# aagbotemi/zk-cryptography

Hardware: AMD Instinct MI355X
Metric: field-evals/s (sumcheck 2^24) + MSM points/s (KZG 2^20) per BASELINE.json; value = the sumcheck prover's field-evals/s, the MSM half is under "msm" (higher is better)
Workload: dtype u32; 1 GPU; 24-var multilinear sumcheck prover (poly_sum + prove), BLS12-381 Fr; field=BLS12-381 Fr (255-bit Montgomery, 8 x u32 limbs); G1 over Fq (381-bit), evals_per_gpu=16777216, exchanges_per_prove=0

## Files before the change

### zk-cryptography_amd/csrc/multifold_kernels.hpp

```cpp
#pragma once
#include "sumcheck_kernels.hpp"
#include "wide_acc.hpp"

namespace zk {

constexpr int MF_MAX_LOGK = 8;
constexpr int MF_CAP_LOGK = 9;

static __global__ __launch_bounds__(MLE_BLOCK) void chunk_sums_kernel(const uint64_t* __restrict__ in, uint32_t chunk,
                                                                      uint64_t* __restrict__ partials) {
    __shared__ Fr red[MLE_BLOCK / 64];
    const uint64_t* base = in + 4 * (size_t)blockIdx.x * chunk;
    Fr s = Fr::zero();
    for (uint32_t j = threadIdx.x; j < chunk; j += 4 * MLE_BLOCK) {
        Fr v[4];
#pragma unroll
        for (int u = 0; u < 4; ++u) v[u] = (j + u * MLE_BLOCK < chunk) ? load_fr(base, j + u * MLE_BLOCK) : Fr::zero();
#pragma unroll
        for (int u = 0; u < 4; ++u) s = s + v[u];
    }
    s = block_reduce_fr(s, red);
    if (threadIdx.x == 0) store_fr(partials, blockIdx.x, s);
}

// ... 37 lines not shown
                                                                         uint64_t* __restrict__ out_mont, uint64_t* __restrict__ out_canon) {
    __shared__ Fr red[MLE_BLOCK / 64];
    const uint64_t* base = in + 4 * (size_t)blockIdx.x * group;
    Fr s = Fr::zero();
    for (uint32_t j = threadIdx.x; j < group; j += 4 * MLE_BLOCK) {
        Fr v[4];
#pragma unroll
        for (int u = 0; u < 4; ++u) v[u] = (j + u * MLE_BLOCK < group) ? load_fr(base, j + u * MLE_BLOCK) : Fr::zero();
#pragma unroll
        for (int u = 0; u < 4; ++u) s = s + v[u];
    }
    s = block_reduce_fr(s, red);
    if (threadIdx.x == 0) {
        if (out_mont) store_fr(out_mont, blockIdx.x, s);
        if (out_canon) store_fr(out_canon, blockIdx.x, fr_from_mont_outlined(s));
    }
}

constexpr int TREE_MAX_LOG = 10;

struct SmallArgs {
    const uint64_t* src;
    uint32_t group;
    uint32_t stride;
    uint32_t canon;
    uint32_t log_n;
    uint32_t n_rounds;
    uint32_t round0;
    uint32_t first;
    FrArg claimed;
    const uint64_t* d_claimed;
    uint64_t* weights_out;
    uint64_t* final_out;
    long long host_delta;
};

constexpr int SMALL_BLOCK = 512;

static __global__ __launch_bounds__(SMALL_BLOCK) void sumcheck_small_kernel(SmallArgs a, SumcheckDev* st,
                                                                            uint64_t* __restrict__ round_polys,
                                                                            uint64_t* __restrict__ challenges) {
    extern __shared__ __attribute__((aligned(16))) unsigned char zk_dyn_lds[];
    __builtin_amdgcn_s_setprio(3);
    ZK_STAMP_AT(0, 40 + a.round0, 0);
    const uint32_t n = 1u << a.log_n;
    Fr* tree0 = reinterpret_cast<Fr*>(zk_dyn_lds);
    Fr* tree1 = tree0 + 2 * n;
    const uint32_t w_all = a.weights_out ? (1u << a.n_rounds) : 0u;
    Fr* w0 = tree1 + n;
    Fr* w1 = w0 + ((a.n_rounds & 1) ? w_all / 2 : w_all);
    const bool grouped = a.group != 0 && a.stride == 0;
    Fr* scratch = w0 + w_all + w_all / 2 + 1;
    Fr* e_sh = scratch + (grouped ? SMALL_BLOCK : 0);
    Fr* r_sh = e_sh + 4;
    if (a.host_delta && a.round0) {
        for (uint32_t i = threadIdx.x; i < 12 * a.round0 + 4; i += SMALL_BLOCK) {
            const uint64_t* p = i < 4 ? st->sum + i : i < 4 + 8 * a.round0 ? round_polys + (i - 4) : challenges + (i - 4 - 8 * a.round0);
            *const_cast<uint64_t*>(p + a.host_delta) = *p;
        }
    }
    if (a.group == 0) {
        for (uint32_t j = threadIdx.x; j < n; j += SMALL_BLOCK) {
            const Fr v = load_fr(a.src, j);
            tree0[n + j] = a.canon ? v : fr_from_mont_outlined(v);
        }
    } else if (a.stride != 0) {
        for (uint32_t j = threadIdx.x; j < n; j += SMALL_BLOCK) {
            Fr s = load_fr(a.src, j);
            for (uint32_t g = 1; g < a.group; g += 8) {
                Fr v[8];
#pragma unroll
                for (int u = 0; u < 8; ++u) if (g + u < a.group) v[u] = load_fr(a.src, (size_t)(g + u) * a.stride + j);
#pragma unroll
                for (int u = 0; u < 8; ++u) if (g + u < a.group) s = s + v[u];
            }
            tree0[n + j] = a.canon ? s : fr_from_mont_outlined(s);
        }
    } else {
        const uint32_t total = n * a.group;
        const uint32_t run = total > (uint32_t)SMALL_BLOCK ? total / SMALL_BLOCK : 1;
        if (threadIdx.x * run < total) {
            Fr s = Fr::zero();
            for (uint32_t g = 0; g < run; ++g) s = s + load_fr(a.src, (size_t)threadIdx.x * run + g);
            scratch[threadIdx.x] = s;
        }
        __syncthreads();
        const uint32_t tpe = a.group / run;
        for (uint32_t j = threadIdx.x; j < n; j += SMALL_BLOCK) {
            Fr s = scratch[j * tpe];
            for (uint32_t g = 1; g < tpe; ++g) s = s + scratch[j * tpe + g];
            tree0[n + j] = a.canon ? s : fr_from_mont_outlined(s);
        }
    }
    if (threadIdx.x == 0 && a.weights_out) {
        Fr one32;
        constexpr uint32_t c[8] = {0xcaaf6b13u, 0x355094eau, 0x69a568efu, 0xf6b10cb3u, 0x40cc3869u, 0xe2c926a6u, 0xed269aadu, 0x736a6d3bu};
#pragma unroll
        for (int i = 0; i < 8; ++i) one32.l[i] = c[i];
        w0[0] = one32;
    }
    __syncthreads();
    for (uint32_t lvl = a.log_n; lvl > 1;) {
        const uint32_t step = lvl - 1 < 3 ? lvl - 1 : 3;
        const uint32_t groups = 1u << (lvl - step);
        for (uint32_t g = threadIdx.x; g < groups; g += SMALL_BLOCK) {
            Fr v[8];
            const uint32_t cnt0 = 1u << step;
#pragma unroll
            for (int i = 0; i < 8; ++i) if ((uint32_t)i < cnt0) v[i] = tree0[(1u << lvl) + g * cnt0 + i];
#pragma unroll
            for (int sft = 1; sft <= 3; ++sft) {
                if ((uint32_t)sft <= step) {
                    const uint32_t cnt = cnt0 >> sft;
#pragma unroll
                    for (int i = 0; i < 4; ++i) {
                        if ((uint32_t)i < cnt) {
                            v[i] = v[2 * i] + v[2 * i + 1];
                            tree0[(1u << (lvl - sft)) + g * cnt + i] = v[i];
                        }
                    }
                }
            }
        }
        __syncthreads();
        lvl -= step;
    }
    const uint32_t wave = threadIdx.x >> 6;
    const bool wave0 = wave == 0;
    uint32_t* kw1 = reinterpret_cast<uint32_t*>(r_sh + 2);
    uint32_t* kw2 = kw1 + 64;
    uint32_t* dig_sh = kw2 + 64;
    uint32_t* flags = dig_sh + 16;
    if (threadIdx.x >= 64 && threadIdx.x < 66 && a.log_n >= 2)
        e_sh[threadIdx.x - 64] = (tree0[6 + threadIdx.x - 64] - tree0[4 + threadIdx.x - 64]).to_mont();
    if (threadIdx.x == 0) {
        flags[0] = 0; flags[1] = 0;
        uint32_t pre[8];
        if (a.first) {
            const Fr sum_c = (a.first == 2) ? fr_from_mont_outlined(fr_from_arg(a.claimed))
                           : (a.first == 3) ? fr_from_mont_outlined(load_fr(a.d_claimed, 0)) : tree0[2] + tree0[3];
#pragma unroll
            for (int i = 0; i < 8; ++i) pre[i] = sum_c.l[7 - i];
        } else {
#pragma unroll
            for (int i = 0; i < 8; ++i) pre[i] = st->transcript.buf[i];
        }
#pragma unroll
        for (int i = 0; i < 8; ++i) dig_sh[8 + i] = pre[i];
    }
    __syncthreads();
    Fr lo = tree0[2], hi = tree0[3];
    uint32_t depth = a.log_n, round = a.round0, n_w = 1;
    ZK_STAMP_AT(0, 40 + a.round0, 1);
    const uint32_t word = threadIdx.x & 15;
    auto schedule_block1 = [&](const uint32_t* prefix, const Fr& lo_c, uint32_t it) {
        const uint32_t w = word < 8 ? prefix[word] : fr_limb_by_lane(lo_c, 15 - word);
        sha256_schedule_rows_to_lds(w, kw1, flags, 4 * it, 1, threadIdx.x < 64 + 16);
    };
    auto schedule_block2 = [&](const Fr& hi_c, uint32_t it) {
        const uint32_t w = word < 8 ? fr_limb_by_lane(hi_c, 7 - word) : (word == 8 ? 0x80000000u : word == 15 ? 96u * 8u : 0u);
        sha256_schedule_rows_to_lds(w, kw2, flags + 1, 4 * it, 0, threadIdx.x < 128 + 16);
    };
    if (a.n_rounds) {
        if (wave == 1) schedule_block1(dig_sh + 8, lo, 0);
        if (wave == 2) schedule_block2(hi, 0);
    }
    uint32_t digest[8];
    constexpr uint32_t FIRST_HELPER = 192, N_HELPERS = SMALL_BLOCK - FIRST_HELPER - 64, OUT_WAVE = 4;
    if (wave == OUT_WAVE) __builtin_amdgcn_s_setprio(0);
    for (uint32_t it = 0; it < a.n_rounds; ++it) {
        Fr* told = (it & 1) ? tree1 : tree0;
        Fr* tnew = (it & 1) ? tree0 : tree1;
        Fr* wold = (it & 1) ? w1 : w0;
        Fr* wnew = (it & 1) ? w0 : w1;
        Fr* eold = e_sh + 2 * (it & 1);
        Fr* enew = e_sh + 2 * ((it & 1) ^ 1);
        const bool absorb_sum = a.first && it == 0;
        if (wave0) {
            ZK_STAMP_AT(0, round, 0);
            uint32_t h[8] = {0x6a09e667u, 0xbb67ae85u, 0x3c6ef372u, 0xa54ff53au, 0x510e527fu, 0x9b05688cu, 0x1f83d9abu, 0x5be0cd19u};
            uint32_t blk[16];
            const uint32_t* pre = dig_sh + 8 * ((it + 1) & 1);
#pragma unroll
            for (int i = 0; i < 8; ++i) { blk[i] = pre[i]; blk[8 + i] = lo.l[7 - i]; }
            ShaSplit sp;
            sp.init();
            uint32_t hs[4];
            sp.split(h, hs);
            sha256_compress_kw_split(sp, hs, blk, kw1, flags, 4 * it);
            ZK_STAMP_AT(0, round, 1);
            sha256_compress_kw_split(sp, hs, nullptr, kw2, flags + 1, 4 * it);
            sp.join(hs, h);
            ZK_STAMP_AT(0, round, 2);
#pragma unroll
            for (int i = 0; i < 8; ++i) digest[i] = h[i];
            Fr c;
#pragma unroll
            for (int i = 0; i < 8; ++i) c.l[i] = h[7 - i];
            c.reduce_once();
            c.reduce_once();
            if (threadIdx.x == 0) {
                r_sh[it & 1] = c;
#pragma unroll
                for (int i = 0; i < 8; ++i) dig_sh[8 * (it & 1) + i] = h[i];
            }
        }
        ZK_STAMP_AT(0, round, 3);
        ZK_STAMP_AT(SMALL_BLOCK - 1, round, 6);
        ZK_STAMP_AT(64, round, 7);
        __syncthreads();
        ZK_STAMP_AT(0, round, 4);
        const Fr c = r_sh[it & 1];
        if (wave0) {
            if (depth >= 2) {
                const uint32_t q = threadIdx.x & 1;
                Fr v = told[4 + q] + fr_mul_outlined(c, eold[q]);
                lo = shfl_fr(v, 0);
                hi = shfl_fr(v, 1);
            }
            ZK_STAMP_AT(0, round, 5);
        } else if (wave <= 2) {
            if (it + 1 < a.n_rounds && depth >= 2) {
                const uint32_t q = wave - 1;
                const Fr v = told[4 + q] + fr_mul_outlined(c, eold[q]);
                if (wave == 1) schedule_block1(dig_sh + 8 * (it & 1), v, it + 1);
                else schedule_block2(v, it + 1);
            }
        } else {
            const Fr r = fr_to_mont_outlined(c);
            const uint32_t helper = wave == OUT_WAVE ? N_HELPERS : wave < OUT_WAVE ? threadIdx.x - FIRST_HELPER : threadIdx.x - FIRST_HELPER - 64;
            if (threadIdx.x == 64 * OUT_WAVE) {
                Fr lo_m = told[2].to_mont(), hi_m = told[3].to_mont();
                if (absorb_sum) {
                    Fr sum_m = (a.first == 2) ? fr_from_arg(a.claimed) : (a.first == 3) ? load_fr(a.d_claimed, 0) : lo_m + hi_m;
                    store_fr(st->sum, 0, sum_m);
                    if (a.host_delta) store_fr(st->sum + a.host_delta, 0, sum_m);
                }
                store_fr(round_polys, 2 * (size_t)round, lo_m);
                store_fr(round_polys, 2 * (size_t)round + 1, hi_m);
                store_fr(challenges, round, r);
                if (a.host_delta) {
                    store_fr(round_polys + a.host_delta, 2 * (size_t)round, lo_m);
                    store_fr(round_polys + a.host_delta, 2 * (size_t)round + 1, hi_m);
                    store_fr(challenges + a.host_delta, round, r);
                }
            }
            const uint32_t nodes = 1u << (depth - 1);
            if (helper >= N_HELPERS - 2 && helper < N_HELPERS && depth >= 3) {
                const uint32_t q = 4 + (helper - (N_HELPERS - 2));
                Fr va = told[q + 4] + r * (told[q + 8] - told[q + 4]);
                Fr vb = told[q + 6] + r * (told[q + 10] - told[q + 6]);
                tnew[q] = va;
                tnew[q + 2] = vb;
                enew[helper - (N_HELPERS - 2)] = (vb - va).to_mont();
            }
            for (uint32_t q = 1 + helper; q < 2 * nodes && helper < N_HELPERS; q += N_HELPERS) {
                if (depth >= 3 && q >= 4 && q < 8) continue;
                const uint32_t p = 1u << (31 - __builtin_clz(q));
                tnew[q] = told[q + p] + r * (told[q + 2 * p] - told[q + p]);
            }
            if (a.weights_out) {
                for (uint32_t b = helper; b < n_w && helper < N_HELPERS; b += N_HELPERS) {
                    Fr w1v = wold[b] * r;
                    wnew[2 * b + 1] = w1v;
                    wnew[2 * b] = wold[b] - w1v;
                }
            }
        }
        n_w <<= 1;
        --depth;
        ++round;
    }
    ZK_STAMP_AT(0, 40 + a.round0, 2);
    __syncthreads();
    if (threadIdx.x == 0 && a.n_rounds) {
        Transcript tr;
        tr.init();
        tr.commit_words8(digest);
        tr.store(&st->transcript);
    }

    if (a.weights_out) {
        Fr* w = (a.n_rounds & 1) ? w1 : w0;
        for (uint32_t b = threadIdx.x; b < n_w; b += SMALL_BLOCK) store_fr(a.weights_out, b, w[b]);
    }
    if (a.final_out) {
        Fr* t = (a.n_rounds & 1) ? tree1 : tree0;
        const uint32_t cnt = 1u << depth;
        for (uint32_t j = threadIdx.x; j < cnt; j += SMALL_BLOCK) store_fr(a.final_out, j, t[cnt + j].to_mont());
    }
}
__host__ __device__ constexpr size_t small_lds_bytes(uint32_t log_n, int weight_rounds, bool grouped) {
    return ((size_t)3 * ((size_t)1 << log_n) + (weight_rounds >= 0 ? 3 * ((size_t)1 << weight_rounds) / 2 : 0u) + 1 +
            (grouped ? SMALL_BLOCK : 0) + 4 + 2) * 32 + (64 + 64 + 16 + 2) * 4;
}

static __global__ __launch_bounds__(MLE_BLOCK) void eq_weights_kernel(PtsArg pts, uint32_t first, uint32_t k,
                                                                      uint64_t* __restrict__ out) {
    const uint32_t b = blockIdx.x * MLE_BLOCK + threadIdx.x;
    if (b >= (1u << k)) return;
    Fr w;
    constexpr uint32_t c[8] = {0xcaaf6b13u, 0x355094eau, 0x69a568efu, 0xf6b10cb3u, 0x40cc3869u, 0xe2c926a6u, 0xed269aadu, 0x736a6d3bu};
#pragma unroll
    for (int i = 0; i < 8; ++i) w.l[i] = c[i];
    const Fr one = Fr::one();
    for (uint32_t i = 0; i < k; ++i) {
        Fr r = fr_from_pts(pts, first + i);
        if (!((b >> (k - 1 - i)) & 1)) r = one - r;
        w = w * r;
    }
    store_fr(out, b, w);
}

static __global__ __launch_bounds__(MLE_BLOCK) void eval_weights_kernel(PtsArg pts, uint32_t k1, uint32_t k2, uint32_t s, uint64_t* __restrict__ w1,
                                                                        uint64_t* __restrict__ wa, uint64_t* __restrict__ wb) {
    size_t b = (size_t)blockIdx.x * MLE_BLOCK + threadIdx.x;
    const size_t n1 = (size_t)1 << k1, na = (size_t)1 << (k2 - s), nb = (size_t)1 << s;
    uint32_t k, first;
    uint64_t* out;
    Fr w = Fr::one();
    if (b < n1) {
        k = k1; first = 0; out = w1;
        constexpr uint32_t c[8] = {0xcaaf6b13u, 0x355094eau, 0x69a568efu, 0xf6b10cb3u, 0x40cc3869u, 0xe2c926a6u, 0xed269aadu, 0x736a6d3bu};
#pragma unroll
        for (int i = 0; i < 8; ++i) w.l[i] = c[i];
    } else if (b < n1 + na) {
        b -= n1; k = k2 - s; first = k1; out = wa;
    } else if (b < n1 + na + nb) {
        b -= n1 + na; k = s; first = k1 + k2 - s; out = wb;
    } else {
        return;
    }
    const Fr one = Fr::one();
    for (uint32_t i = 0; i < k; ++i) {
        Fr r = fr_from_pts(pts, first + i);
        if (!((b >> (k - 1 - i)) & 1)) r = one - r;
        w = w * r;
    }
    store_fr(out, b, w);
}
static __global__ __launch_bounds__(MLE_BLOCK) void sum_records_kernel(const uint64_t* __restrict__ records, uint32_t n, uint64_t* __restrict__ out) {
    __shared__ Fr red[MLE_BLOCK / 64];
    Fr s = Fr::zero();
    for (uint32_t i = threadIdx.x; i < n; i += 4 * MLE_BLOCK) {
        Fr v[4];
#pragma unroll
        for (int u = 0; u < 4; ++u) v[u] = (i + u * MLE_BLOCK < n) ? load_fr(records, i + u * MLE_BLOCK) : Fr::zero();
// ... 11 lines not shown
                                                                uint64_t* __restrict__ partials) {
    constexpr int TG = 64 / G;
    extern __shared__ __attribute__((aligned(16))) unsigned char zk_dyn_lds[];
    Fr* w_lds = reinterpret_cast<Fr*>(zk_dyn_lds);
    Fr* part = w_lds + (1u << k);
    const uint32_t n_terms = 1u << k;
    for (uint32_t b = threadIdx.x; b < n_terms; b += blockDim.x) w_lds[b] = load_fr(weights, b);
    __syncthreads();
    const uint32_t lane = threadIdx.x & 63;
    const uint32_t wave = threadIdx.x >> 6;
    const uint32_t n_waves = blockDim.x >> 6;
    const uint32_t slice = wave * TG + lane / G;
    const uint32_t per = n_terms / (n_waves * TG);
    const uint32_t oj = lane % G;
    const size_t j = (size_t)blockIdx.x * G + oj;
    WideAcc acc;
    acc.clear();
    const uint32_t b0 = slice * per;
    const uint64_t* p = in + 4 * ((size_t)b0 * m + j);
    const size_t row = 4 * m;
    for (uint32_t t = 0; t < per; t += DEPTH) {
        Fr v[DEPTH];
#pragma unroll
        for (int u = 0; u < DEPTH; ++u) if (t + u < per) v[u] = NT ? load_fr_nt(p + (size_t)(t + u) * row) : load_fr(p + (size_t)(t + u) * row, 0);
#pragma unroll
        for (int u = 0; u < DEPTH; ++u) if (t + u < per) acc.mac(w_lds[b0 + t + u], v[u]);
    }
    Fr o = wide_reduce(acc.lo, acc.hi);
#pragma unroll
    for (int d = 32; d >= G; d >>= 1) o = o + shfl_down_fr(o, d);
    if (wave != 0 && lane < G) part[(wave - 1) * G + lane] = o;
    __syncthreads();
    if (wave == 0) {
        if (lane < G) {
            for (uint32_t w2 = 1; w2 < n_waves; ++w2) o = o + part[(w2 - 1) * G + lane];
            store_fr(out, j, o);
        } else {
            o = Fr::zero();
        }
        Fr s = wave_reduce_fr(o);
        if (lane == 0) store_fr(partials, blockIdx.x, s);
    }
}

static __global__ __launch_bounds__(MLE_BLOCK) void slice_sums_kernel(const uint64_t* __restrict__ in, uint32_t ny, uint32_t m,
                                                               uint64_t* __restrict__ out) {
    const uint32_t j = blockIdx.x * MLE_BLOCK + threadIdx.x;
    if (j >= m) return;
    Fr s = load_fr(in, j);
    for (uint32_t y = 1; y < ny; ++y) s = s + load_fr(in, (size_t)y * m + j);
    store_fr(out, j, fr_to_mont_outlined(s));
}

constexpr int BF_BLOCK = 1024;
static __global__ __launch_bounds__(BF_BLOCK) void blockfold_kernel(const uint64_t* __restrict__ in, uint32_t m, uint32_t log_ow,
                                                                    uint32_t per, const uint64_t* __restrict__ weights,
                                                                    uint64_t* __restrict__ partial) {
    __shared__ Fr part[BF_BLOCK];
    const uint32_t ow = 1u << log_ow, sl_cnt = BF_BLOCK >> log_ow;
    const uint32_t o = threadIdx.x & (ow - 1), sl = threadIdx.x >> log_ow;
    const uint32_t c = blockIdx.x * ow + o;
    const uint32_t b0 = (blockIdx.y * sl_cnt + sl) * per;
    WideAcc acc;
    acc.clear();
    for (uint32_t u = 0; u < per; u += 2) {
        Fr v0 = load_fr(in, (size_t)(b0 + u) * m + c), w0 = load_fr(weights, b0 + u);
        Fr v1 = v0, w1 = w0;
        const bool two = u + 1 < per;
        if (two) { v1 = load_fr(in, (size_t)(b0 + u + 1) * m + c); w1 = load_fr(weights, b0 + u + 1); }
        acc.mac(w0, v0);
        if (two) acc.mac(w1, v1);
    }
    part[threadIdx.x] = wide_reduce(acc.lo, acc.hi);
    __syncthreads();
    for (uint32_t half = sl_cnt >> 1; half >= 1; half >>= 1) {
        if (sl < half) part[threadIdx.x] = part[threadIdx.x] + part[threadIdx.x + (half << log_ow)];
        __syncthreads();
    }
    if (sl == 0) store_fr(partial, (size_t)blockIdx.y * m + c, fr_from_mont_outlined(part[o]));
}

}
```

### zk-cryptography_amd/csrc/transcript.hpp

```cpp
#pragma once
#include "fp.hpp"

namespace zk {

struct Sha256State {
    uint32_t h[8];
    uint32_t buf[16];
    uint32_t fill;
    uint32_t pad_;
    uint64_t len;
};

__device__ __forceinline__ uint32_t rotr32(uint32_t x, int n) { return __builtin_rotateright32(x, n); }

static __constant__ uint32_t SHA256_K[64] = {
    0x428a2f98, 0x71374491, 0xb5c0fbcf, 0xe9b5dba5, 0x3956c25b, 0x59f111f1, 0x923f82a4, 0xab1c5ed5,
    0xd807aa98, 0x12835b01, 0x243185be, 0x550c7dc3, 0x72be5d74, 0x80deb1fe, 0x9bdc06a7, 0xc19bf174,
    0xe49b69c1, 0xefbe4786, 0x0fc19dc6, 0x240ca1cc, 0x2de92c6f, 0x4a7484aa, 0x5cb0a9dc, 0x76f988da,
    0x983e5152, 0xa831c66d, 0xb00327c8, 0xbf597fc7, 0xc6e00bf3, 0xd5a79147, 0x06ca6351, 0x14292967,
    0x27b70a85, 0x2e1b2138, 0x4d2c6dfc, 0x53380d13, 0x650a7354, 0x766a0abb, 0x81c2c92e, 0x92722c85,
    0xa2bfe8a1, 0xa81a664b, 0xc24b8b70, 0xc76c51a3, 0xd192e819, 0xd6990624, 0xf40e3585, 0x106aa070,
    0x19a4c116, 0x1e376c08, 0x2748774c, 0x34b0bcb5, 0x391c0cb3, 0x4ed8aa4a, 0x5b9cca4f, 0x682e6ff3,
    0x748f82ee, 0x78a5636f, 0x84c87814, 0x8cc70208, 0x90befffa, 0xa4506ceb, 0xbef9a3f7, 0xc67178f2};

// ... 315 lines not shown
    }
    sp.join(hs, h);
}

__device__ __forceinline__ void sha256_compress_wave(uint32_t (&h)[8], const uint32_t (&blk)[16], uint32_t* lds) {
    const uint32_t i = threadIdx.x & 15;
    uint32_t w = blk[0];
#pragma unroll
    for (int k = 1; k < 16; ++k) w = i == (uint32_t)k ? blk[k] : w;
    sha256_schedule_rows_to_lds(w, lds, nullptr, 0u, 0u, (threadIdx.x & 63) < 16);
    __builtin_amdgcn_fence(__ATOMIC_ACQ_REL, "workgroup");
    ShaSplit sp;
    sp.init();
    uint32_t hs[4];
    sp.split(h, hs);
    sha256_rounds_block_split(sp, hs, lds);
    sp.join(hs, h);
    __builtin_amdgcn_fence(__ATOMIC_ACQ_REL, "workgroup");
}

__device__ __noinline__ Fr fr_mul_outlined(Fr a, Fr b) { return a * b; }
__device__ __noinline__ Fr fr_from_mont_outlined(Fr a) {
    uint32_t x[9];
#pragma unroll
    for (int i = 0; i < 8; ++i) x[i] = a.l[i];
    x[8] = 0;
#pragma unroll
    for (int i = 0; i < 8; ++i) {
        const uint32_t m = FrParams::mul_inv(x[0]);
        uint64_t c = ((uint64_t)m * FrParams::p(0) + x[0]) >> 32;
#pragma unroll
        for (int j = 1; j < 8; ++j) {
            uint64_t s = (uint64_t)m * FrParams::p(j) + x[j] + c;
            x[j - 1] = (uint32_t)s;
            c = s >> 32;
        }
        uint64_t s = (uint64_t)x[8] + c;
        x[7] = (uint32_t)s;
        x[8] = (uint32_t)(s >> 32);
    }
    Fr r;
#pragma unroll
    for (int i = 0; i < 8; ++i) r.l[i] = x[i];
    r.reduce_once();
    return r;
}
__device__ __forceinline__ Fr fr_to_mont_outlined(const Fr& a) {
    Fr r2;
#pragma unroll
    for (int i = 0; i < Fr::N; ++i) r2.l[i] = FrParams::r2(i);
    return fr_mul_outlined(a, r2);
}

struct Transcript {
    uint32_t h[8];
    uint32_t buf[16];
    uint32_t fill_words;
    uint64_t len;

    __device__ __forceinline__ void init() {
        h[0] = 0x6a09e667; h[1] = 0xbb67ae85; h[2] = 0x3c6ef372; h[3] = 0xa54ff53a;
        h[4] = 0x510e527f; h[5] = 0x9b05688c; h[6] = 0x1f83d9ab; h[7] = 0x5be0cd19;
        fill_words = 0;
        len = 0;
#pragma unroll
        for (int i = 0; i < 16; ++i) buf[i] = 0;
    }
    __device__ __forceinline__ void load(const Sha256State* s) {
#pragma unroll
        for (int i = 0; i < 8; ++i) h[i] = s->h[i];
#pragma unroll
        for (int i = 0; i < 16; ++i) buf[i] = s->buf[i];
        fill_words = s->fill >> 2;
        len = s->len;
    }
    __device__ __forceinline__ void store(Sha256State* s) const {
#pragma unroll
        for (int i = 0; i < 8; ++i) s->h[i] = h[i];
#pragma unroll
        for (int i = 0; i < 16; ++i) s->buf[i] = buf[i];
        s->fill = fill_words << 2;
        s->len = len;
    }
    __device__ __forceinline__ void commit_words8(const uint32_t (&wds)[8]) {
        if (fill_words == 0) {
#pragma unroll
            for (int i = 0; i < 8; ++i) buf[i] = wds[i];
            fill_words = 8;
        } else {
#pragma unroll
            for (int i = 0; i < 8; ++i) buf[8 + i] = wds[i];
            sha256_compress(h, buf);
            fill_words = 0;
        }
        len += 32;
    }
    __device__ __forceinline__ void commit_canonical(const Fr& c) {
        uint32_t wds[8];
#pragma unroll
        for (int i = 0; i < 8; ++i) wds[i] = c.l[7 - i];
        commit_words8(wds);
    }
    __device__ __forceinline__ void commit_fr(const Fr& v_mont) {
        Fr c = fr_from_mont_outlined(v_mont);
        uint32_t wds[8];
#pragma unroll
// ... 63 lines not shown
```

### zk-cryptography_amd/csrc/zkhip.hip

```cpp
#include "../../include/zkhip.h"

#include <hip/hip_runtime.h>

#include <algorithm>
#include <cstdio>
#include <cstdlib>
#include <cstring>
#include <map>
#include <string>
#include <vector>

#include "ctx.hpp"
#include "host_util.hpp"
#include "mle_kernels.hpp"
#include "sumcheck_kernels.hpp"
#include "multifold_kernels.hpp"
#include "mfma_fold.hpp"
#include "tunables.hpp"

using namespace zk;

static int g_last_hip = 0;
extern "C" int zkhip_version(void) { return 1; }

// ... 431 lines not shown
extern "C" int zkhip_circuit_add_mult_mle(zkhip_ctx* c, const uint8_t* h_gate_type, const uint32_t* h_in0, const uint32_t* h_in1,
                                          size_t n_gates, uint32_t layer_index, uint64_t* d_add, uint64_t* d_mul) {
    if (!c || !d_add || !d_mul || (n_gates && (!h_gate_type || !h_in0 || !h_in1))) return ZKHIP_ERR_ARG;
    if (layer_index > 12) return ZKHIP_ERR_SHAPE;
    const size_t size = zkhip_gkr_mle_size(layer_index);
    const uint32_t shift = layer_index + 1;
    for (size_t g = 0; g < n_gates; ++g) {
        const size_t idx = (g << (2 * shift)) | ((size_t)h_in0[g] << shift) | h_in1[g];
        if (idx >= size) return ZKHIP_ERR_INDEX;
    }
    ZK_TRY(c->activate());
    ZK_HIP(c, hipMemsetAsync(d_add, 0, 32 * size, c->stream));
    ZK_HIP(c, hipMemsetAsync(d_mul, 0, 32 * size, c->stream));
    if (n_gates == 0) return ZKHIP_OK;
    uint32_t* d_gates = nullptr;
    ZK_TRY(upload_gates(c, h_gate_type, h_in0, h_in1, n_gates, &d_gates));
    hipLaunchKernelGGL(wiring_ones_kernel, dim3(mle_grid(n_gates)), dim3(MLE_BLOCK), 0, c->stream, d_gates, n_gates, shift, d_add, d_mul);
    ZK_HIP(c, hipGetLastError());
    ZK_HIP(c, hipStreamSynchronize(c->stream));
    return ZKHIP_OK;
}

static inline uint32_t stage_k(size_t cur_n) {
    if (cur_n <= ((size_t)1 << TREE_MAX_LOG)) return 0;
    const uint32_t lg = log2_exact(cur_n);
    uint32_t k = lg - 8;
    if (k > MF_MAX_LOGK) k = MF_MAX_LOGK;
    return k;
}
static inline uint32_t overlapped_min_log() {
    static const uint32_t v = (uint32_t)zk::env::read(zk::env::OVERLAP_MIN_LOG); return v;
}
static inline bool overlapped_plan(size_t n) { return is_pow2(n) && n >= ((size_t)1 << overlapped_min_log()) && n <= ((size_t)1 << 24); }
static inline bool overlapped_shard(size_t n) { return is_pow2(n) && n >= ((size_t)1 << 19) && n <= ((size_t)1 << 24); }
static inline uint32_t overlapped_k2(size_t n) { return std::min<uint32_t>(TREE_MAX_LOG, log2_exact(n) - 8 - 3); }
extern "C" int zkhip_sumcheck_plan_log_blocks(size_t n) {
    if (!is_pow2(n)) return 0;
    return overlapped_plan(n) ? (int)(log2_exact(n) - 8) : (int)stage_k(n);
}

static int launch_small(zkhip_ctx* c, const SmallArgs& a, SumcheckDev* st, uint64_t* d_rp, uint64_t* d_ch, size_t min_lds = 0,
                        hipStream_t stream = nullptr) {
    if (!stream) stream = c->stream;
    if (a.log_n > (uint32_t)TREE_MAX_LOG || a.n_rounds > a.log_n) return ZKHIP_ERR_SHAPE;
    const size_t lds = std::max(small_lds_bytes(a.log_n, a.weights_out ? (int)a.n_rounds : -1, a.group != 0 && a.stride == 0), min_lds);
    if (lds > 160 * 1024) return ZKHIP_ERR_SHAPE;
    ZK_TRY(c->allow_big_lds((const void*)sumcheck_small_kernel, 160 * 1024));
    ProfScope ps(c, "sumcheck_small", 0.0, stream);
    hipLaunchKernelGGL(sumcheck_small_kernel, dim3(1), dim3(SMALL_BLOCK), lds, stream, a, st, d_rp, d_ch);
    ZK_HIP(c, hipGetLastError());
    return ZKHIP_OK;
}

struct BlockfoldShape { uint32_t log_ow, per, ny; };
static inline bool blockfold_shape(uint32_t m, uint32_t k, BlockfoldShape* sh) {
    const uint32_t log_m = log2_exact(m);
    sh->log_ow = std::max<uint32_t>(std::min<uint32_t>(log_m, 5), k < 10 ? 10 - k : 0);
    if (sh->log_ow > log_m) return false;
    const uint32_t sl_cnt = (uint32_t)BF_BLOCK >> sh->log_ow;
    const uint32_t terms = 1u << k;
    sh->per = std::min<uint32_t>(4, terms / sl_cnt);
    sh->ny = terms / (sh->per * sl_cnt);
    return true;
}
static int launch_blockfold(zkhip_ctx* c, hipStream_t stream, const uint64_t* in, uint32_t m, uint32_t k, const uint64_t* d_w,
                            uint64_t* d_partial, uint32_t* n_slices) {
    BlockfoldShape sh;
    if (!blockfold_shape(m, k, &sh)) return ZKHIP_ERR_SHAPE;
    const uint32_t log_ow = sh.log_ow, per = sh.per, ny = sh.ny, terms = 1u << k;
    ProfScope ps(c, "blockfold", 32.0 * (double)m * terms, stream);
    hipLaunchKernelGGL(blockfold_kernel, dim3(m >> log_ow, ny), dim3(BF_BLOCK), 0, stream, in, m, log_ow, per, d_w, d_partial);
    ZK_HIP(c, hipGetLastError());
    *n_slices = ny;
    return ZKHIP_OK;
}
static int launch_fine_sums(zkhip_ctx* c, const uint64_t* d_evals, size_t n, uint32_t lb, uint64_t* d_fine, uint64_t* d_chunk,
                            hipStream_t stream = nullptr) {
    if (!stream) stream = c->stream;
    const size_t blk = n >> lb, n_chunks = n / FINE_CHUNK;
    uint64_t* first = blk == (size_t)FINE_CHUNK ? d_fine : d_chunk;
    {
        ProfScope ps(c, "fine_sums", 32.0 * (double)n, stream);
        static const size_t lds = (size_t)zk::env::read(zk::env::FINE_LDS);
        if (lds > 64 * 1024) ZK_TRY(c->allow_big_lds((const void*)fine_sums_kernel, 158 * 1024));
        hipLaunchKernelGGL(fine_sums_kernel, dim3((unsigned)((n_chunks + 7) / 8)), dim3(MLE_BLOCK), lds, stream, d_evals, n_chunks, first);
    }
    if (first != d_fine)
        hipLaunchKernelGGL(group_sums_wg_kernel, dim3(1u << lb), dim3(MLE_BLOCK), 0, stream, first, (uint32_t)(blk / FINE_CHUNK), d_fine, (uint64_t*)nullptr);
    ZK_HIP(c, hipGetLastError());
    return ZKHIP_OK;
}

static int block_sums_impl(zkhip_ctx* c, const uint64_t* d_evals, size_t n, uint32_t log_blocks, uint64_t* d_out, uint64_t* h_total, bool want_total);
extern "C" int zkhip_mle_block_sums(zkhip_ctx* c, const uint64_t* d_evals, size_t n, uint32_t log_blocks,
                                    uint64_t* d_out, uint64_t* h_total) {
    return block_sums_impl(c, d_evals, n, log_blocks, d_out, h_total, true);
}
extern "C" int zkhip_mle_block_sums_deferred(zkhip_ctx* c, const uint64_t* d_evals, size_t n, uint32_t log_blocks, uint64_t* d_out) {
    return block_sums_impl(c, d_evals, n, log_blocks, d_out, nullptr, false);
}
extern "C" int zkhip_mle_block_sums_total(zkhip_ctx* c, uint64_t* d_block_sums, uint32_t log_blocks, uint64_t* h_total) {
    if (!c || !d_block_sums || !h_total || log_blocks > 16) return ZKHIP_ERR_ARG;
    ZK_TRY(c->activate());
    const uint32_t hi = log_blocks / 2, lo = log_blocks - hi;
    uint64_t* tmp = c->small_u64(ZK_SMALL_PARTIALS);
    hipLaunchKernelGGL(group_sums_wg_kernel, dim3(1u << hi), dim3(MLE_BLOCK), 0, c->stream, d_block_sums, 1u << lo, tmp, (uint64_t*)nullptr);
    hipLaunchKernelGGL(group_sums_wg_kernel, dim3(1), dim3(MLE_BLOCK), 0, c->stream, tmp, 1u << hi, d_block_sums + 4 * ((size_t)1 << log_blocks), (uint64_t*)nullptr);
    ZK_HIP(c, hipGetLastError());
    ZK_HIP(c, hipMemcpyAsync(c->pinned_u64(ZK_PIN_RES), d_block_sums + 4 * ((size_t)1 << log_blocks), 32, hipMemcpyDeviceToHost, c->stream));
    ZK_HIP(c, hipStreamSynchronize(c->stream));
    std::memcpy(h_total, c->pinned_u64(ZK_PIN_RES), 32);
    return ZKHIP_OK;
}
static int block_sums_impl(zkhip_ctx* c, const uint64_t* d_evals, size_t n, uint32_t log_blocks, uint64_t* d_out, uint64_t* h_total, bool want_total) {
    if (!c || !d_evals || !d_out) return ZKHIP_ERR_ARG;
    if (!is_pow2(n) || log_blocks > 16 || ((size_t)1 << log_blocks) > n) return ZKHIP_ERR_SHAPE;
    ZK_TRY(c->activate());
    const size_t m = n >> log_blocks;
    if (log_blocks > (uint32_t)MF_CAP_LOGK) {
        if (m < (size_t)FINE_CHUNK) return ZKHIP_ERR_SHAPE;
        uint64_t* d_chunk = nullptr;
        if (m > (size_t)FINE_CHUNK) { ZK_TRY(c->reserve_ws((n / FINE_CHUNK) * 32)); d_chunk = (uint64_t*)c->ws.ptr; }
        ZK_TRY(launch_fine_sums(c, d_evals, n, log_blocks, d_out, d_chunk));
        if (want_total) {
            const uint32_t k1 = overlapped_plan(n) && log_blocks == log2_exact(n) - 8 ? log_blocks - overlapped_k2(n) : 8;
            int cs = 0;
// ... 691 lines not shown
```

Baseline: 53.02 billion field-evals/s.

## Split challenge multiply across 8 lanes with precomputed limb-weighted constants

Removes the serial challenge reduction and full Montgomery multiply from the critical path after each SHA-256 digest. Each of 8 lanes multiplies one raw digest limb by a precomputed per-limb-scaled copy of the fold difference, the partial products are summed with DPP cross-lane add chains, and a Barrett-style reduction follows. Helper waves now precompute the 8 scaled constants per node for the next round using DPP lane differences. This lowers the latency of the sequential per-round transcript chain, at the cost of hand-written inline assembly, more LDS slots, and correctness that depends on the carry and bound handling being right.

Result: no change. 52.84 billion field-evals/s (-0.3%).

```diff
diff --git a/zk-cryptography_amd/csrc/multifold_kernels.hpp b/zk-cryptography_amd/csrc/multifold_kernels.hpp
--- a/zk-cryptography_amd/csrc/multifold_kernels.hpp
+++ b/zk-cryptography_amd/csrc/multifold_kernels.hpp
@@ -113,7 +113,6 @@
     const bool grouped = a.group != 0 && a.stride == 0;
     Fr* scratch = w0 + w_all + w_all / 2 + 1;
     Fr* e_sh = scratch + (grouped ? SMALL_BLOCK : 0);
-    Fr* r_sh = e_sh + 4;
     if (a.host_delta && a.round0) {
         for (uint32_t i = threadIdx.x; i < 12 * a.round0 + 4; i += SMALL_BLOCK) {
             const uint64_t* p = i < 4 ? st->sum + i : i < 4 + 8 * a.round0 ? round_polys + (i - 4) : challenges + (i - 4 - 8 * a.round0);
@@ -188,12 +187,14 @@
     }
     const uint32_t wave = threadIdx.x >> 6;
     const bool wave0 = wave == 0;
-    uint32_t* kw1 = reinterpret_cast<uint32_t*>(r_sh + 2);
+    uint32_t* kw1 = reinterpret_cast<uint32_t*>(e_sh + 32);
     uint32_t* kw2 = kw1 + 64;
     uint32_t* dig_sh = kw2 + 64;
     uint32_t* flags = dig_sh + 16;
-    if (threadIdx.x >= 64 && threadIdx.x < 66 && a.log_n >= 2)
-        e_sh[threadIdx.x - 64] = (tree0[6 + threadIdx.x - 64] - tree0[4 + threadIdx.x - 64]).to_mont();
+    if (threadIdx.x >= 64 && threadIdx.x < 80 && a.log_n >= 2) {
+        const uint32_t q = (threadIdx.x - 64) >> 3;
+        e_sh[threadIdx.x - 64] = fr_mul_outlined(tree0[6 + q] - tree0[4 + q], fr_late_table_const(threadIdx.x & 7));
+    }
     if (threadIdx.x == 0) {
         flags[0] = 0; flags[1] = 0;
         uint32_t pre[8];
@@ -234,8 +235,8 @@
         Fr* tnew = (it & 1) ? tree0 : tree1;
         Fr* wold = (it & 1) ? w1 : w0;
         Fr* wnew = (it & 1) ? w0 : w1;
-        Fr* eold = e_sh + 2 * (it & 1);
-        Fr* enew = e_sh + 2 * ((it & 1) ^ 1);
+        Fr* eold = e_sh + 16 * (it & 1);
+        Fr* enew = e_sh + 16 * ((it & 1) ^ 1);
         const bool absorb_sum = a.first && it == 0;
         if (wave0) {
             ZK_STAMP_AT(0, round, 0);
@@ -255,13 +256,7 @@
             ZK_STAMP_AT(0, round, 2);
 #pragma unroll
             for (int i = 0; i < 8; ++i) digest[i] = h[i];
-            Fr c;
-#pragma unroll
-            for (int i = 0; i < 8; ++i) c.l[i] = h[7 - i];
-            c.reduce_once();
-            c.reduce_once();
             if (threadIdx.x == 0) {
-                r_sh[it & 1] = c;
 #pragma unroll
                 for (int i = 0; i < 8; ++i) dig_sh[8 * (it & 1) + i] = h[i];
             }
@@ -271,23 +266,29 @@
         ZK_STAMP_AT(64, round, 7);
         __syncthreads();
         ZK_STAMP_AT(0, round, 4);
-        const Fr c = r_sh[it & 1];
+        const uint32_t* dig = dig_sh + 8 * (it & 1);
+        const uint32_t limb = threadIdx.x & 7;
         if (wave0) {
             if (depth >= 2) {
-                const uint32_t q = threadIdx.x & 1;
-                Fr v = told[4 + q] + fr_mul_outlined(c, eold[q]);
-                lo = shfl_fr(v, 0);
-                hi = shfl_fr(v, 1);
+                const uint32_t q = (threadIdx.x >> 3) & 1;
+                const Fr v = fr_late_product8(dig[7 - limb], eold[8 * q + limb], told[4 + q]);
+                lo = readlane_fr(v, 0);
+                hi = readlane_fr(v, 8);
             }
             ZK_STAMP_AT(0, round, 5);
         } else if (wave <= 2) {
             if (it + 1 < a.n_rounds && depth >= 2) {
                 const uint32_t q = wave - 1;
-                const Fr v = told[4 + q] + fr_mul_outlined(c, eold[q]);
-                if (wave == 1) schedule_block1(dig_sh + 8 * (it & 1), v, it + 1);
+                const Fr v = readlane_fr(fr_late_product8(dig[7 - limb], eold[8 * q + limb], told[4 + q]), 0);
+                if (wave == 1) schedule_block1(dig, v, it + 1);
                 else schedule_block2(v, it + 1);
             }
         } else {
+            Fr c;
+#pragma unroll
+            for (int i = 0; i < 8; ++i) c.l[i] = dig[7 - i];
+            c.reduce_once();
+            c.reduce_once();
             const Fr r = fr_to_mont_outlined(c);
             const uint32_t helper = wave == OUT_WAVE ? N_HELPERS : wave < OUT_WAVE ? threadIdx.x - FIRST_HELPER : threadIdx.x - FIRST_HELPER - 64;
             if (threadIdx.x == 64 * OUT_WAVE) {
@@ -307,13 +308,14 @@
                 }
             }
             const uint32_t nodes = 1u << (depth - 1);
-            if (helper >= N_HELPERS - 2 && helper < N_HELPERS && depth >= 3) {
-                const uint32_t q = 4 + (helper - (N_HELPERS - 2));
-                Fr va = told[q + 4] + r * (told[q + 8] - told[q + 4]);
-                Fr vb = told[q + 6] + r * (told[q + 10] - told[q + 6]);
-                tnew[q] = va;
-                tnew[q + 2] = vb;
-                enew[helper - (N_HELPERS - 2)] = (vb - va).to_mont();
+            if (helper >= N_HELPERS - 16 && helper < N_HELPERS && depth >= 3) {
+                const uint32_t j = helper - (N_HELPERS - 16), q = j >> 3;
+                const Fr kc = fr_late_table_const(limb);
+                const uint32_t node = 4 + q + 2 * (j & 1);
+                const Fr nv = told[node + 4] + fr_mul_outlined(r, told[node + 8] - told[node + 4]);
+                if (limb < 2) tnew[node] = nv;
+                const Fr diff = dpp_fr<0xF5, 0xf>(nv) - dpp_fr<0xA0, 0xf>(nv);
+                enew[8 * q + limb] = fr_mul_outlined(diff, kc);
             }
             for (uint32_t q = 1 + helper; q < 2 * nodes && helper < N_HELPERS; q += N_HELPERS) {
                 if (depth >= 3 && q >= 4 && q < 8) continue;
@@ -353,7 +355,7 @@
 }
 __host__ __device__ constexpr size_t small_lds_bytes(uint32_t log_n, int weight_rounds, bool grouped) {
     return ((size_t)3 * ((size_t)1 << log_n) + (weight_rounds >= 0 ? 3 * ((size_t)1 << weight_rounds) / 2 : 0u) + 1 +
-            (grouped ? SMALL_BLOCK : 0) + 4 + 2) * 32 + (64 + 64 + 16 + 2) * 4;
+            (grouped ? SMALL_BLOCK : 0) + 32) * 32 + (64 + 64 + 16 + 2) * 4;
 }
 
 static __global__ __launch_bounds__(MLE_BLOCK) void eq_weights_kernel(PtsArg pts, uint32_t first, uint32_t k,
diff --git a/zk-cryptography_amd/csrc/transcript.hpp b/zk-cryptography_amd/csrc/transcript.hpp
--- a/zk-cryptography_amd/csrc/transcript.hpp
+++ b/zk-cryptography_amd/csrc/transcript.hpp
@@ -391,6 +391,146 @@
     return fr_mul_outlined(a, r2);
 }
 
+#define ZK_DPP_ADDC(I, CTRL) "v_addc_co_u32_dpp %" #I ", vcc, %" #I ", %" #I ", vcc " CTRL " row_mask:0xf bank_mask:0xf\n\t"
+#define ZK_DPP_ADD10(X, CTRL)                                                                                          \
+    asm volatile("s_nop 1\n\t"                                                                                         \
+                 "v_add_co_u32_dpp %0, vcc, %0, %0 " CTRL " row_mask:0xf bank_mask:0xf\n\t"                            \
+                 ZK_DPP_ADDC(1, CTRL) ZK_DPP_ADDC(2, CTRL) ZK_DPP_ADDC(3, CTRL) ZK_DPP_ADDC(4, CTRL) ZK_DPP_ADDC(5, CTRL)  \
+                 ZK_DPP_ADDC(6, CTRL) ZK_DPP_ADDC(7, CTRL) ZK_DPP_ADDC(8, CTRL) ZK_DPP_ADDC(9, CTRL)                   \
+                 : "+v"(X[0]), "+v"(X[1]), "+v"(X[2]), "+v"(X[3]), "+v"(X[4]), "+v"(X[5]), "+v"(X[6]), "+v"(X[7]), "+v"(X[8]), "+v"(X[9]) \
+                 :                                                                                                     \
+                 : "vcc");
+__device__ __forceinline__ void sub_chain9(uint32_t (&r)[9], const uint32_t (&b)[9]) {
+    asm("v_sub_co_u32 %0, vcc, %0, %9\n\t"
+        "v_subb_co_u32 %1, vcc, %1, %10, vcc\n\t"
+        "v_subb_co_u32 %2, vcc, %2, %11, vcc\n\t"
+        "v_subb_co_u32 %3, vcc, %3, %12, vcc\n\t"
+        "v_subb_co_u32 %4, vcc, %4, %13, vcc\n\t"
+        "v_subb_co_u32 %5, vcc, %5, %14, vcc\n\t"
+        "v_subb_co_u32 %6, vcc, %6, %15, vcc\n\t"
+        "v_subb_co_u32 %7, vcc, %7, %16, vcc\n\t"
+        "v_subb_co_u32 %8, vcc, %8, %17, vcc"
+        : "+v"(r[0]), "+v"(r[1]), "+v"(r[2]), "+v"(r[3]), "+v"(r[4]), "+v"(r[5]), "+v"(r[6]), "+v"(r[7]), "+v"(r[8])
+        : "v"(b[0]), "v"(b[1]), "v"(b[2]), "v"(b[3]), "v"(b[4]), "v"(b[5]), "v"(b[6]), "v"(b[7]), "v"(b[8])
+        : "vcc");
+}
+__device__ __forceinline__ void sub_chain8_up1(uint32_t (&r)[9], const uint32_t (&b)[8]) {
+    asm("v_sub_co_u32 %0, vcc, %0, %8\n\t"
+        "v_subb_co_u32 %1, vcc, %1, %9, vcc\n\t"
+        "v_subb_co_u32 %2, vcc, %2, %10, vcc\n\t"
+        "v_subb_co_u32 %3, vcc, %3, %11, vcc\n\t"
+        "v_subb_co_u32 %4, vcc, %4, %12, vcc\n\t"
+        "v_subb_co_u32 %5, vcc, %5, %13, vcc\n\t"
+        "v_subb_co_u32 %6, vcc, %6, %14, vcc\n\t"
+        "v_subb_co_u32 %7, vcc, %7, %15, vcc"
+        : "+v"(r[1]), "+v"(r[2]), "+v"(r[3]), "+v"(r[4]), "+v"(r[5]), "+v"(r[6]), "+v"(r[7]), "+v"(r[8])
+        : "v"(b[0]), "v"(b[1]), "v"(b[2]), "v"(b[3]), "v"(b[4]), "v"(b[5]), "v"(b[6]), "v"(b[7])
+        : "vcc");
+}
+__device__ __forceinline__ void add_chain8_into9(uint32_t (&r)[9], const uint32_t (&b)[8]) {
+    asm("v_add_co_u32 %0, vcc, %0, %9\n\t"
+        "v_addc_co_u32 %1, vcc, %1, %10, vcc\n\t"
+        "v_addc_co_u32 %2, vcc, %2, %11, vcc\n\t"
+        "v_addc_co_u32 %3, vcc, %3, %12, vcc\n\t"
+        "v_addc_co_u32 %4, vcc, %4, %13, vcc\n\t"
+        "v_addc_co_u32 %5, vcc, %5, %14, vcc\n\t"
+        "v_addc_co_u32 %6, vcc, %6, %15, vcc\n\t"
+        "v_addc_co_u32 %7, vcc, %7, %16, vcc\n\t"
+        "v_addc_co_u32 %8, vcc, 0, %8, vcc"
+        : "+v"(r[0]), "+v"(r[1]), "+v"(r[2]), "+v"(r[3]), "+v"(r[4]), "+v"(r[5]), "+v"(r[6]), "+v"(r[7]), "+v"(r[8])
+        : "v"(b[0]), "v"(b[1]), "v"(b[2]), "v"(b[3]), "v"(b[4]), "v"(b[5]), "v"(b[6]), "v"(b[7])
+        : "vcc");
+}
+__device__ __forceinline__ void cond_sub_chain9(uint32_t (&r)[9], const uint32_t (&m)[8]) {
+    uint32_t t0, t1, t2, t3, t4, t5, t6, t7, t8;
+    asm("v_sub_co_u32 %9, vcc, %0, %18\n\t"
+        "v_subb_co_u32 %10, vcc, %1, %19, vcc\n\t"
+        "v_subb_co_u32 %11, vcc, %2, %20, vcc\n\t"
+        "v_subb_co_u32 %12, vcc, %3, %21, vcc\n\t"
+        "v_subb_co_u32 %13, vcc, %4, %22, vcc\n\t"
+        "v_subb_co_u32 %14, vcc, %5, %23, vcc\n\t"
+        "v_subb_co_u32 %15, vcc, %6, %24, vcc\n\t"
+        "v_subb_co_u32 %16, vcc, %7, %25, vcc\n\t"
+        "v_subbrev_co_u32 %17, vcc, 0, %8, vcc\n\t"
+        "v_cndmask_b32 %0, %9, %0, vcc\n\t"
+        "v_cndmask_b32 %1, %10, %1, vcc\n\t"
+        "v_cndmask_b32 %2, %11, %2, vcc\n\t"
+        "v_cndmask_b32 %3, %12, %3, vcc\n\t"
+        "v_cndmask_b32 %4, %13, %4, vcc\n\t"
+        "v_cndmask_b32 %5, %14, %5, vcc\n\t"
+        "v_cndmask_b32 %6, %15, %6, vcc\n\t"
+        "v_cndmask_b32 %7, %16, %7, vcc"
+        : "+v"(r[0]), "+v"(r[1]), "+v"(r[2]), "+v"(r[3]), "+v"(r[4]), "+v"(r[5]), "+v"(r[6]), "+v"(r[7]), "+v"(r[8]),
+          "=&v"(t0), "=&v"(t1), "=&v"(t2), "=&v"(t3), "=&v"(t4), "=&v"(t5), "=&v"(t6), "=&v"(t7), "=&v"(t8)
+        : "v"(m[0]), "v"(m[1]), "v"(m[2]), "v"(m[3]), "v"(m[4]), "v"(m[5]), "v"(m[6]), "v"(m[7])
+        : "vcc");
+}
+__device__ __forceinline__ Fr fr_late_product8(uint32_t di, const Fr& mi, const Fr& a) {
+    uint32_t x[10];
+    uint64_t acc = 0;
+#pragma unroll
+    for (int j = 0; j < 8; ++j) {
+        acc = (uint64_t)mi.l[j] * di + (acc >> 32);
+        x[j] = (uint32_t)acc;
+    }
+    x[8] = (uint32_t)(acc >> 32);
+    x[9] = 0;
+    ZK_DPP_ADD10(x, "row_shl:1")
+    ZK_DPP_ADD10(x, "row_shl:2")
+    ZK_DPP_ADD10(x, "row_shl:4")
+    const uint32_t t_lo = __builtin_amdgcn_alignbit(x[8], x[7], 2), t_hi = __builtin_amdgcn_alignbit(x[9], x[8], 2);
+    constexpr uint32_t MU_LO = 0xd54253b7u, MU_HI = 0x8u;
+    const uint64_t pa = (uint64_t)t_lo * MU_LO;
+    const uint64_t pb = (uint64_t)t_hi * MU_LO + (pa >> 32);
+    const uint64_t pc = (uint64_t)t_lo * MU_HI + (uint32_t)pb;
+    const uint64_t qe = (uint64_t)t_hi * MU_HI + (pb >> 32) + (pc >> 32);
+    const uint32_t q_lo = (uint32_t)qe, q_hi = (uint32_t)(qe >> 32);
+    uint32_t t[9], y[9], z[8];
+#pragma unroll
+    for (int i = 0; i < 9; ++i) t[i] = x[i];
+    acc = 0;
+#pragma unroll
+    for (int j = 0; j < 8; ++j) {
+        acc = (uint64_t)q_lo * FrParams::p(j) + (acc >> 32);
+        y[j] = (uint32_t)acc;
+    }
+    y[8] = (uint32_t)(acc >> 32);
+    acc = 0;
+#pragma unroll
+    for (int j = 0; j < 8; ++j) {
+        acc = (uint64_t)q_hi * FrParams::p(j) + (acc >> 32);
+        z[j] = (uint32_t)acc;
+    }
+    sub_chain9(t, y);
+    sub_chain8_up1(t, z);
+    add_chain8_into9(t, a.l);
+    constexpr uint32_t R2X[8] = {0x00000002u, 0xfffffffeu, 0xfffcb7fdu, 0xa77b4805u, 0x1343b00au, 0x6673b010u, 0x533afa90u, 0xe7db4ea6u};
+    uint32_t m2[8];
+#pragma unroll
+    for (int i = 0; i < 8; ++i) m2[i] = R2X[i];
+    cond_sub_chain9(t, m2);
+    Fr r;
+#pragma unroll
+    for (int i = 0; i < 8; ++i) r.l[i] = t[i];
+    r.reduce_once();
+    return r;
+}
+static __constant__ uint32_t FR_LATE_TABLE_K[8][8] = {
+    {0xfffffffeu, 0x00000001u, 0x00034802u, 0x5884b7fau, 0xecbc4ff5u, 0x998c4fefu, 0xacc5056fu, 0x1824b159u},
+    {0xcaaf6b13u, 0x355094eau, 0x69a568efu, 0xf6b10cb3u, 0x40cc3869u, 0xe2c926a6u, 0xed269aadu, 0x736a6d3bu},
+    {0x0121c884u, 0xc98da28eu, 0xc7363c67u, 0xe6f4f4a0u, 0xe92e7df1u, 0xb2d6ebc4u, 0x9d26242au, 0x19ae5794u},
+    {0xc74a2349u, 0x39d7a53au, 0x605fbb45u, 0x5394c74du, 0x088943e5u, 0x1563f13du, 0x3c5771fbu, 0x03913033u},
+    {0xf81f712du, 0xcf2ab21bu, 0xac0a600du, 0x9277efb8u, 0x7369510au, 0x7abbe568u, 0xd4843acbu, 0x2dbeaf1fu},
+    {0x9afbc14cu, 0x5d23afe0u, 0x2b0e40d0u, 0x1deef9adu, 0x203ba106u, 0xe07e784du, 0xa251b319u, 0x562ca75au},
+    {0x41b4528fu, 0x59476ebcu, 0x43fcc152u, 0xc5a30cb2u, 0x40ccbd72u, 0x2b34e639u, 0xca247088u, 0x1e179025u},
+    {0xbd8c85feu, 0x8427cc90u, 0x0fe630beu, 0xc8ff7852u, 0x27715045u, 0x2b4d2b66u, 0xe5a19691u, 0x05753400u}};
+__device__ __forceinline__ Fr fr_late_table_const(uint32_t i) {
+    Fr k;
+#pragma unroll
+    for (int j = 0; j < 8; ++j) k.l[j] = FR_LATE_TABLE_K[i][j];
+    return k;
+}
+
 struct Transcript {
     uint32_t h[8];
     uint32_t buf[16];
```

## Reshape blockfold into 256-thread blocks with wave-shuffle reduction and target grid fill

Applied to the files above, without the earlier changes.

Shrinks the blockfold workgroup from 1024 to 256 threads with a fixed output width of 8 columns. The host shape function now picks the y-split to aim for about 256 workgroups, capped at 8 partial tables. The per-thread MAC loop is fully unrolled with all loads issued before the multiply-accumulates. The LDS tree reduction with a barrier per level is replaced by wave shuffles plus one LDS exchange across waves. This is meant to raise occupancy and cut barrier and LDS overhead, at the cost of more partial slices for the later slice-sum pass; a static_assert checks that the partial buffers still fit.

Result: faster. 52.76 billion field-evals/s before, 53.69 billion field-evals/s after, median of 6 (+1.8%).

```diff
diff --git a/zk-cryptography_amd/csrc/multifold_kernels.hpp b/zk-cryptography_amd/csrc/multifold_kernels.hpp
--- a/zk-cryptography_amd/csrc/multifold_kernels.hpp
+++ b/zk-cryptography_amd/csrc/multifold_kernels.hpp
@@ -471,32 +471,64 @@
     store_fr(out, j, fr_to_mont_outlined(s));
 }
 
-constexpr int BF_BLOCK = 1024;
-static __global__ __launch_bounds__(BF_BLOCK) void blockfold_kernel(const uint64_t* __restrict__ in, uint32_t m, uint32_t log_ow,
+constexpr int BF_BLOCK = 256;
+constexpr int BF_LOG_OW = 3;
+constexpr int BF_SLICES = BF_BLOCK >> BF_LOG_OW;
+constexpr int BF_MAX_PER = 4;
+constexpr int BF_MAX_NY = 8;
+constexpr int BF_TARGET_WGS = 256;
+
+struct BlockfoldShape { uint32_t log_ow, sl, per, ny; };
+__host__ __device__ constexpr bool blockfold_shape(uint32_t m, uint32_t k, BlockfoldShape* sh) {
+    if (m == 0 || (m & (m - 1)) != 0 || (m >> BF_LOG_OW) == 0) return false;
+    if (k == 0 || k > 10) return false;
+    const uint32_t terms = 1u << k, wgx = m >> BF_LOG_OW;
+    const uint32_t fill = wgx >= (uint32_t)BF_TARGET_WGS ? 1u : (uint32_t)BF_TARGET_WGS / wgx;
+    const uint32_t forced = (terms + BF_SLICES * BF_MAX_PER - 1) / (BF_SLICES * BF_MAX_PER);
+    uint32_t ny = fill > forced ? fill : forced;
+    if (ny > (uint32_t)BF_MAX_NY) ny = BF_MAX_NY;
+    if (ny > terms) ny = terms;
+    const uint32_t range = terms / ny;
+    sh->log_ow = BF_LOG_OW;
+    sh->sl = range < (uint32_t)BF_SLICES ? range : (uint32_t)BF_SLICES;
+    sh->per = range / sh->sl;
+    sh->ny = ny;
+    return true;
+}
+
+static __global__ __launch_bounds__(BF_BLOCK) void blockfold_kernel(const uint64_t* __restrict__ in, uint32_t m, uint32_t sl_cnt,
                                                                     uint32_t per, const uint64_t* __restrict__ weights,
                                                                     uint64_t* __restrict__ partial) {
-    __shared__ Fr part[BF_BLOCK];
-    const uint32_t ow = 1u << log_ow, sl_cnt = BF_BLOCK >> log_ow;
-    const uint32_t o = threadIdx.x & (ow - 1), sl = threadIdx.x >> log_ow;
-    const uint32_t c = blockIdx.x * ow + o;
+    constexpr uint32_t OW = 1u << BF_LOG_OW, WAVES = BF_BLOCK / 64;
+    __shared__ Fr part[(WAVES - 1) * OW];
+    const uint32_t lane = threadIdx.x & 63, wave = threadIdx.x >> 6;
+    const uint32_t o = lane & (OW - 1), sl = wave * (64 / OW) + (lane >> BF_LOG_OW);
+    const uint32_t c = blockIdx.x * OW + o;
     const uint32_t b0 = (blockIdx.y * sl_cnt + sl) * per;
-    WideAcc acc;
-    acc.clear();
-    for (uint32_t u = 0; u < per; u += 2) {
-        Fr v0 = load_fr(in, (size_t)(b0 + u) * m + c), w0 = load_fr(weights, b0 + u);
-        Fr v1 = v0, w1 = w0;
-        const bool two = u + 1 < per;
-        if (two) { v1 = load_fr(in, (size_t)(b0 + u + 1) * m + c); w1 = load_fr(weights, b0 + u + 1); }
-        acc.mac(w0, v0);
-        if (two) acc.mac(w1, v1);
-    }
-    part[threadIdx.x] = wide_reduce(acc.lo, acc.hi);
+    Fr r = Fr::zero();
+    if (sl < sl_cnt) {
+        Fr v[BF_MAX_PER], w[BF_MAX_PER];
+#pragma unroll
+        for (int u = 0; u < BF_MAX_PER; ++u) {
+            if ((uint32_t)u < per) { v[u] = load_fr(in, (size_t)(b0 + u) * m + c); w[u] = load_fr(weights, b0 + u); }
+        }
+        WideAcc acc;
+        acc.clear();
+#pragma unroll
+        for (int u = 0; u < BF_MAX_PER; ++u) {
+            if ((uint32_t)u < per) acc.mac(w[u], v[u]);
+        }
+        r = wide_reduce(acc.lo, acc.hi);
+    }
+#pragma unroll
+    for (int d = 32; d >= (int)OW; d >>= 1) r = r + shfl_down_fr(r, d);
+    if (wave != 0 && lane < OW) part[(wave - 1) * OW + lane] = r;
     __syncthreads();
-    for (uint32_t half = sl_cnt >> 1; half >= 1; half >>= 1) {
-        if (sl < half) part[threadIdx.x] = part[threadIdx.x] + part[threadIdx.x + (half << log_ow)];
-        __syncthreads();
-    }
-    if (sl == 0) store_fr(partial, (size_t)blockIdx.y * m + c, fr_from_mont_outlined(part[o]));
-}
-
-}
+    if (wave == 0 && lane < OW) {
+#pragma unroll
+        for (uint32_t w2 = 1; w2 < WAVES; ++w2) r = r + part[(w2 - 1) * OW + lane];
+        store_fr(partial, (size_t)blockIdx.y * m + c, fr_from_mont_outlined(r));
+    }
+}
+
+}
diff --git a/zk-cryptography_amd/csrc/zkhip.hip b/zk-cryptography_amd/csrc/zkhip.hip
--- a/zk-cryptography_amd/csrc/zkhip.hip
+++ b/zk-cryptography_amd/csrc/zkhip.hip
@@ -507,26 +507,24 @@
     return ZKHIP_OK;
 }
 
-struct BlockfoldShape { uint32_t log_ow, per, ny; };
-static inline bool blockfold_shape(uint32_t m, uint32_t k, BlockfoldShape* sh) {
-    const uint32_t log_m = log2_exact(m);
-    sh->log_ow = std::max<uint32_t>(std::min<uint32_t>(log_m, 5), k < 10 ? 10 - k : 0);
-    if (sh->log_ow > log_m) return false;
-    const uint32_t sl_cnt = (uint32_t)BF_BLOCK >> sh->log_ow;
-    const uint32_t terms = 1u << k;
-    sh->per = std::min<uint32_t>(4, terms / sl_cnt);
-    sh->ny = terms / (sh->per * sl_cnt);
+constexpr bool blockfold_fits(uint32_t m, uint32_t k_max, uint32_t room) {
+    for (uint32_t k = 1; k <= k_max; ++k) {
+        BlockfoldShape sh = {};
+        if (!blockfold_shape(m, k, &sh) || sh.ny * m > room || sh.sl * sh.per * sh.ny != (1u << k)) return false;
+    }
     return true;
 }
+static_assert(blockfold_fits(256, 6, 2048) && blockfold_fits(512, 6, 2048) && blockfold_fits(1024, 6, 2048) && blockfold_fits(256, 10, 32 * 256),
+              "blockfold_shape: more partial tables than the prover's buffers hold");
 static int launch_blockfold(zkhip_ctx* c, hipStream_t stream, const uint64_t* in, uint32_t m, uint32_t k, const uint64_t* d_w,
                             uint64_t* d_partial, uint32_t* n_slices) {
     BlockfoldShape sh;
     if (!blockfold_shape(m, k, &sh)) return ZKHIP_ERR_SHAPE;
-    const uint32_t log_ow = sh.log_ow, per = sh.per, ny = sh.ny, terms = 1u << k;
+    const uint32_t terms = 1u << k;
     ProfScope ps(c, "blockfold", 32.0 * (double)m * terms, stream);
-    hipLaunchKernelGGL(blockfold_kernel, dim3(m >> log_ow, ny), dim3(BF_BLOCK), 0, stream, in, m, log_ow, per, d_w, d_partial);
-    ZK_HIP(c, hipGetLastError());
-    *n_slices = ny;
+    hipLaunchKernelGGL(blockfold_kernel, dim3(m >> sh.log_ow, sh.ny), dim3(BF_BLOCK), 0, stream, in, m, sh.sl, sh.per, d_w, d_partial);
+    ZK_HIP(c, hipGetLastError());
+    *n_slices = sh.ny;
     return ZKHIP_OK;
 }
 static int launch_fine_sums(zkhip_ctx* c, const uint64_t* d_evals, size_t n, uint32_t lb, uint64_t* d_fine, uint64_t* d_chunk,
```
